# sequential-dexterity/SeqDex

Measured on AMD Instinct MI355X. Metric: env-steps/sec BlockAssemblyGraspSim num_envs=1024/GPU, higher is better.
Workload: dtype f32; 1 GPU; BlockAssemblyGraspSim num_envs=1024 per GPU, fp32, PPO MLP policy [1024,512,256], horizon 8, minibatch_size 4, mini_epochs 5, central value (configs[1]); step=one rl_games epoch = 8 env steps x num_envs + full PPO update, global_envs=1024, piles=synthetic settled piles, 64 per brick-type group, policy=random init, seed 22+rank

## Files before the change

### seqdex_amd/csrc/sdxp_persist.hip

```cpp
#include <cstddef>
#include <cstdlib>

#include "sdx_common.h"
#include "sdxp_device.h"
#include "sdxp_launch.h"
#include "sdxp_persist_lds.h"
#include "sdxp_persist_exchange.h"
#include "sdxp_persist_sums.h"
#include "sdxp_persist_adam.h"
#include "sdxp_persist_tails.h"
#include "sdxp_persist_phase_d.h"

__device__ __forceinline__ const float* obs_rows(const SdxpDev& D, int mb) { return D.mb_obs + (size_t)mb * MB * D.obs_dim; }
__device__ __forceinline__ const float* cvx_rows(const SdxpDev& D, int mb, int mini_epoch) {
  return (mini_epoch == 0 ? D.cvx0 : D.cvx1) + (size_t)mb * MB * ST;
}

template <bool SINGLE>
__global__ __launch_bounds__(NTH, 2) void k_update_persistent(SdxpDev D, int total_steps, const float* gx0_tab, unsigned* failflag, int stamps, int fault) {
  extern __shared__ __attribute__((aligned(16))) char smem_raw[];
  PLds& S = *reinterpret_cast<PLds*>(smem_raw);
  int tid = threadIdx.x, wave = tid >> 6, lane = tid & 63, g = blockIdx.x;
  int r0w, h0, n0, r1w, q1, r1, c2c, c2n, he, hrow, hk;
  auto refresh = [&]() {
    int t = threadIdx.x, b = blockIdx.x;
    asm volatile("" : "+v"(t));
    asm volatile("" : "+s"(b));
    tid = t; lane = t & 63; wave = __builtin_amdgcn_readfirstlane(t >> 6); g = b;
    r0w = wave >> 1; h0 = wave & 1; n0 = 4 * g + r0w;
    r1w = wave >> 2; q1 = wave & 3; r1 = 2 * g + r1w;
    c2c = (t >> 5) & 1; c2n = 32 * (t >> 6) + (t & 31);
    he = HPC * g + t; hrow = he >> 8; hk = he & (U2 - 1);
  };
  refresh();
#define TS(i) if (stamps && g == (stamps >> 8) && tid == 0) { const long long t_ = __builtin_amdgcn_s_memtime(); S.tacc[i] += t_ - S.tlast; S.tlast = t_; }
  if (tid < 32) S.tacc[tid] = 0;
  if (tid == 0) S.fail = 0;
  if (tid == 0) S.tlast = __builtin_amdgcn_s_memtime();
  const int A = ACT;
  u64* const LL = D.ll;
  const __amdgpu_buffer_rsrc_t LQ = lq_rsrc(D.ll);

  float w0a[I0A], m0a[I0A], v0a[I0A], w0c[I0A], m0c[I0A], v0c[I0A], w0v[I0V], m0v[I0V], v0v[I0V];
  float w1[3][4], m1[3][4], v1[3][4];
  float c1[3][4], cm1[3][4], cv1[3][4];
  float w2[3], m2[3], v2[3];
  float c2[3], cm2[3], cv2[3];
  float hw = 0.0f, hm = 0.0f, hv = 0.0f;

  auto ldm = [&](const float* p, size_t o) -> float { return SINGLE ? 0.0f : p[o]; };
  auto P_of = [&](int net) -> float* { return net == 2 ? D.cv : D.ac; };
  auto M_of = [&](int net) -> float* { return net == 2 ? D.cv_m : D.ac_m; };
  auto V_of = [&](int net) -> float* { return net == 2 ? D.cv_v : D.ac_v; };
  auto woff = [&](int net, int l) -> size_t { return net == 0 ? D.off.a_w[l] : net == 1 ? D.off.c_w[l] : D.coff.w[l]; };
  auto boff = [&](int net, int l) -> size_t { return net == 0 ? D.off.a_b[l] : net == 1 ? D.off.c_b[l] : D.coff.b[l]; };
  auto head_woff = [&](int row) -> size_t { return row < A ? D.off.mu_w + (size_t)row * U2 : (row == A ? D.off.v_w : D.coff.v_w); };
  auto head_boff = [&](int row) -> size_t { return row < A ? D.off.mu_b + row : (row == A ? D.off.v_b : D.coff.v_b); };
  auto head_net = [&](int row) -> int { return row < A ? 0 : (row == A ? 1 : 2); };
  auto k_w1 = [&](int i) -> int { return q1 * 256 + lane + 64 * i; };
  auto o_w0 = [&](int net, int k) -> size_t { return woff(net, 0) + (size_t)n0 * D.obs_dim + k; };
  auto o_w1 = [&](int net, int i) -> size_t { return woff(net, 1) + (size_t)r1 * U0 + q1 * 256 + lane + 64 * i; };
  auto o_hw = [&]() -> size_t { return head_woff(hrow) + hk; };

#pragma unroll
  for (int i = 0; i < I0A; ++i) {
    const int kk = lane + 64 * i, k = h0 * H0A + kk;
    const bool ok = kk < H0A && k < D.obs_dim;
    const size_t oa = o_w0(0, k), oc = o_w0(1, k);
    w0a[i] = ok ? D.ac[oa] : 0.0f; m0a[i] = ok ? ldm(D.ac_m, oa) : 0.0f; v0a[i] = ok ? ldm(D.ac_v, oa) : 0.0f;
    w0c[i] = ok ? D.ac[oc] : 0.0f; m0c[i] = ok ? ldm(D.ac_m, oc) : 0.0f; v0c[i] = ok ? ldm(D.ac_v, oc) : 0.0f;
  }
#pragma unroll
  for (int i = 0; i < I0V; ++i) {
    const int kk = lane + 64 * i, k = h0 * H0V + kk;
    const bool ok = kk < H0V;
    const size_t o = woff(2, 0) + (size_t)n0 * ST + k;
    w0v[i] = ok ? D.cv[o] : 0.0f; m0v[i] = ok ? ldm(D.cv_m, o) : 0.0f; v0v[i] = ok ? ldm(D.cv_v, o) : 0.0f;
  }
#pragma unroll
  for (int net = 0; net < 3; ++net) {
#pragma unroll
    for (int i = 0; i < 4; ++i) {
      const size_t o = o_w1(net, i);
      w1[net][i] = P_of(net)[o]; m1[net][i] = ldm(M_of(net), o); v1[net][i] = ldm(V_of(net), o);
    }
#pragma unroll
    for (int c = 0; c < 4; ++c) {
      const size_t o = woff(net, 1) + (size_t)tid * U0 + 4 * g + c;
      c1[net][c] = P_of(net)[o]; cm1[net][c] = ldm(M_of(net), o); cv1[net][c] = ldm(V_of(net), o);
    }
    {
      const size_t o = woff(net, 2) + (size_t)g * U1 + wave * 64 + lane;
      w2[net] = P_of(net)[o]; m2[net] = ldm(M_of(net), o); v2[net] = ldm(V_of(net), o);
    }
    {
      const size_t o = woff(net, 2) + (size_t)c2n * U1 + 2 * g + c2c;
      c2[net] = P_of(net)[o]; cm2[net] = ldm(M_of(net), o); cv2[net] = ldm(V_of(net), o);
    }
  }
  if (tid < HPC) {
    const int net = head_net(hrow);
    const size_t o = o_hw();
    hw = P_of(net)[o]; hm = ldm(M_of(net), o); hv = ldm(V_of(net), o);
  }
  __shared__ float s_b2[3][32];
  auto bias_load = [&](int net, size_t o) { S.bias[tid] = P_of(net)[o]; S.bias_m[tid] = ldm(M_of(net), o); S.bias_v[tid] = ldm(V_of(net), o); };
  if (tid < BIAS_L1) { const int net = (tid - BIAS_L0) / 4, w = (tid - BIAS_L0) % 4; bias_load(net, boff(net, 0) + 4 * g + w); }
  else if (tid < BIAS_L2) { const int net = (tid - BIAS_L1) / 2, r = (tid - BIAS_L1) % 2; bias_load(net, boff(net, 1) + 2 * g + r); }
  else if (tid < BIAS_HEAD) { const int net = tid - BIAS_L2; bias_load(net, boff(net, 2) + g); }
  else if (tid < BIAS_HEAD + A + 2) { const int row = tid - BIAS_HEAD; bias_load(head_net(row), head_boff(row)); }
  else if (tid >= T_LOGSTD && tid < T_LOGSTD + A) {
    const int a = tid - T_LOGSTD;
    const size_t o = D.off.logstd + a;
    s_b2[0][a] = D.ac[o]; s_b2[1][a] = ldm(D.ac_m, o); s_b2[2][a] = ldm(D.ac_v, o);
  }
// ... 9 lines not shown
  float g0a[I0A], g0c[I0A], g0v[I0V];
#pragma unroll
  for (int i = 0; i < I0A; ++i) { g0a[i] = 0.0f; g0c[i] = 0.0f; }
#pragma unroll
  for (int i = 0; i < I0V; ++i) g0v[i] = 0.0f;
  for (int i = tid; i < MB * OBS; i += NTH) (&S.obs[0][0])[i] = 0.0f;
  __syncthreads();

  auto load_rows = [&](int mb_, int me_) {
    auto uni = [](const float* q) -> const float* { unsigned long long a = (unsigned long long)q; asm volatile("" : "+s"(a)); return (const float*)a; };
    const float* o = uni(obs_rows(D, mb_));
    const float* c = uni(cvx_rows(D, mb_, me_));
    const unsigned odim = D.obs_dim;
    if constexpr (!SINGLE) {
      const float* gt = uni(gx0_tab + (size_t)mb_ * GX0_STRIDE);
      if (wave == NWV - 1 && lane < 32)
        __builtin_amdgcn_global_load_lds(SDX_AS_GLOBAL(gt + (lane < 16 ? GX0_OBS + lane : (me_ == 0 ? GX0_CVX0 : GX0_CVX1) + (lane - 16))), SDX_AS_LDS(&S.gx0[0][0]), 4, 0, 0);
    }
    if (odim == OBS) {
      static_assert(offsetof(PLds, cvx) == sizeof(float) * MB * OBS && (MB * OBS) % 4 == 0 && (MB * ST) % 4 == 0, "obs and cvx images are adjacent 16-byte runs");
      constexpr int PO = MB * OBS / 4, PA = PO + MB * ST / 4;
      char* l0 = reinterpret_cast<char*>(&S.obs[0][0]);
#pragma unroll
      for (int j = 0; j < (PA + NTH - 1) / NTH; ++j) {
        const int pc = tid + NTH * j;
        if (pc < PA) {
          const float* src = pc < PO ? o + 4 * pc : c + 4 * (pc - PO);
          __builtin_amdgcn_global_load_lds(SDX_AS_GLOBAL(src), SDX_AS_LDS(l0 + (wave + NWV * j) * 1024), 16, 0, 0);
        }
      }
      return;
    }
#pragma unroll
    for (int s = 0; s < MB; ++s) {
      const float* orow = uni(o + s * odim);
      const float* crow = uni(c + s * ST);
      if ((unsigned)tid < odim) __builtin_amdgcn_global_load_lds(SDX_AS_GLOBAL(orow + (unsigned)tid), SDX_AS_LDS(&S.obs[s][wave * 64]), 4, 0, 0);
      __builtin_amdgcn_global_load_lds(SDX_AS_GLOBAL(crow + (unsigned)tid), SDX_AS_LDS(&S.cvx[s][wave * 64]), 4, 0, 0);
      if (tid + NTH < ST) __builtin_amdgcn_global_load_lds(SDX_AS_GLOBAL(crow + NTH + (unsigned)tid), SDX_AS_LDS(&S.cvx[s][NTH]), 4, 0, 0);
    }
  };
  if (total_steps > 0) load_rows(SINGLE ? gctl->mb_index : 0, SINGLE ? gctl->mini_epoch : 0);
  u32x4 pg0[4];
  bool pg0_issued = false;
  for (int step = 0; step <= total_steps; ++step) {
    SDX_LDS_BARRIER();
    if (S.fail) return;
    if (fault && g == NWG - 1 && step == 3) return;
    refresh();
    const bool last = step == total_steps;
    const int mbi = SINGLE ? gctl->mb_index : step % D.num_minibatches, mini_epoch = SINGLE ? gctl->mini_epoch : step / D.num_minibatches;
    const unsigned tag = tag_base + (unsigned)step + 1u, tag_prev = tag_base + (unsigned)step;
    if (pending) {
      float nr0 = S.n2rest[0], nr1 = S.n2rest[1], nr2 = S.n2rest[2];
      float ac_lr_bc1 = S.scal[SC_AC_LR_BC1], ac_isq = S.scal[SC_AC_ISQ], cv_lr_bc1 = S.scal[SC_CV_LR_BC1], cv_isq = S.scal[SC_CV_ISQ];
      float w0[4], w1[4], w2[4];
      lq_take_or_gather<4>(pg0_issued, pg0, LQ, LQ_G0 + lane, 64, tag_prev, w0, w1, w2, failflag, S.fail);
      float n2[3];
      n2[0] = (w0[0] + w0[1]) + (w0[2] + w0[3]); n2[1] = (w1[0] + w1[1]) + (w1[2] + w1[3]); n2[2] = (w2[0] + w2[1]) + (w2[2] + w2[3]);
#pragma unroll
      for (int net = 0; net < 3; ++net) n2[net] = wave_sum(n2[net]);
      SDX_PIN4X(nr0, nr1, nr2, ac_lr_bc1); SDX_PIN3X(ac_isq, cv_lr_bc1, cv_isq);
      n2[0] += nr0; n2[1] += nr1; n2[2] += nr2;
      const float ac_gn = __builtin_amdgcn_sqrtf(n2[0] + n2[1]), cv_gn = __builtin_amdgcn_sqrtf(n2[2]);
      const float gs_ac = D.truncate_grads ? fminf(1.0f, D.grad_norm * __builtin_amdgcn_rcpf(ac_gn + 1e-6f)) : 1.0f;
      const float gs_cv = D.truncate_grads ? fminf(1.0f, D.grad_norm * __builtin_amdgcn_rcpf(cv_gn + 1e-6f)) : 1.0f;
      if (tid == 0) { S.ctl.ac_gn = ac_gn; S.ctl.cv_gn = cv_gn; S.scal[SC_AC_GSCALE] = gs_ac; S.scal[SC_CV_GSCALE] = gs_cv; }
      TS(0)
#pragma unroll
      for (int i = 0; i < I0A; ++i) {
        adam1p(w0a[i], g0a[i] * gs_ac, m0a[i], v0a[i], ac_lr_bc1, ac_isq);
        adam1p(w0c[i], g0c[i] * gs_ac, m0c[i], v0c[i], ac_lr_bc1, ac_isq);
      }
#pragma unroll
      for (int i = 0; i < I0V; ++i) adam1p(w0v[i], g0v[i] * gs_cv, m0v[i], v0v[i], cv_lr_bc1, cv_isq);
      if (tid < BIAS_L1) {
        const int net = (tid - BIAS_L0) / 4;
        float gg = 0.0f;
        for (int s = 0; s < MB; ++s) gg += S.dyown[net][s][DY_L0 + (tid - BIAS_L0) % 4];
        adam_bias(S, StepScal{gs_ac, gs_cv, ac_lr_bc1, ac_isq, cv_lr_bc1, cv_isq}, tid, net, gg);
      }
      TS(1)
    }
    if (!last) {
      SDX_WAIT_VMCNT0();
      __syncthreads();
      float pa[MB], pc[MB], pv[MB];
#pragma unroll
      for (int s = 0; s < MB; ++s) { pa[s] = 0.0f; pc[s] = 0.0f; pv[s] = 0.0f; }
#pragma unroll
      for (int i = 0; i < I0A; ++i) {
        const int kk = lane + 64 * i, k = h0 * H0A + kk;
        if (kk < H0A) {
#pragma unroll
          for (int s = 0; s < MB; ++s) { const float x = S.obs[s][k]; pa[s] += w0a[i] * x; pc[s] += w0c[i] * x; }
        }
      }
#pragma unroll
      for (int i = 0; i < I0V; ++i) {
        const int kk = lane + 64 * i, k = h0 * H0V + kk;
        if (kk < H0V) {
#pragma unroll
          for (int s = 0; s < MB; ++s) pv[s] += w0v[i] * S.cvx[s][k];
        }
      }
      {
        float v[3 * MB], u[3];
#pragma unroll
        for (int s = 0; s < MB; ++s) { v[0 * MB + s] = pa[s]; v[1 * MB + s] = pc[s]; v[2 * MB + s] = pv[s]; }
        wave_sums<3 * MB>(v, u, lane);
        fpart_store(S, u, wave, lane);
      }
      __syncthreads();
      if (wave == 0) {
        float y[3];
        fwd_tail<0>(S, lane, y);
        if (tid < MB * 4) lq_store(LQ, LQ_X1 + (unsigned)(tid / 4) * U0 + 4 * g + tid % 4, y[0], y[1], y[2], tag);
      }
      TS(2)
    }
    refresh();
    if (pending) {
      const StepScal sc = step_scal(S);
      adam_l1_ahead(S, sc, q1 * 256 + lane, 4 * g, r1w, tid, w1, m1, v1, c1, cm1, cv1, [](int, int, float) {});
      if (tid >= BIAS_L1 && tid < BIAS_L2) {
        const int net = (tid - BIAS_L1) / 2;
        float gg = 0.0f;
        for (int s = 0; s < MB; ++s) gg += S.dyown[net][s][DY_L1 + (tid - BIAS_L1) % 2];
        adam_bias(S, sc, tid, net, gg);
      }
    }
    TS(3)
    if (!last) {
      __syncthreads();
      {
        float v0[8], v1[8], v2[8];
        if (!lq_gather<8>(LQ, LQ_X1 + tid, NTH, tag, v0, v1, v2, failflag)) S.fail = 1;
        image_store(S.x1, v0, v1, v2, tid);
      }
      TS(4)
      __syncthreads();
      {
        float q[3 * MB], u[3];
#pragma unroll
        for (int net = 0; net < 3; ++net) {
#pragma unroll
          for (int s = 0; s < MB; ++s) q[net * MB + s] = 0.0f;
#pragma unroll
          for (int i = 0; i < 4; ++i) {
            const int k = k_w1(i);
#pragma unroll
            for (int s = 0; s < MB; ++s) q[net * MB + s] += w1[net][i] * S.x1[net][s][k];
          }
        }
        wave_sums<3 * MB>(q, u, lane);
        fpart_store(S, u, wave, lane);
      }
      __syncthreads();
      if (wave == 0) {
        float y[3];
        fwd_tail<1>(S, lane, y);
        if (tid < MB * 2) lq_store(LQ, LQ_X2 + (unsigned)(tid / 2) * U1 + 2 * g + tid % 2, y[0], y[1], y[2], tag);
      }
      TS(5)
    }
    refresh();
    u32x4 px2[4];
    bool px2_issued = false;
    if (pending) {
      const StepScal sc = step_scal(S);
      float dep = 0.0f;
#pragma unroll
      for (int net = 0; net < 3; ++net) {
        if (net == 2 && !last) { lq_peek<4>(LQ, LQ_X2 + tid, NTH, px2); px2_issued = true; }
        const float gs = sc.gs(net), lrb = sc.lrb(net), isq = sc.isq(net);
        float d2r[MB], dn2[MB];
        const int o_n = opaque(c2n, dep);
#pragma unroll
        for (int s = 0; s < MB; ++s) { d2r[s] = S.dyown[net][s][DY_L2] * gs; dn2[s] = S.dy2[net][s][o_n] * gs; }
        {
          const int k = opaque(wave * 64 + lane, dep);
          float gg = 0.0f;
#pragma unroll
          for (int s = 0; s < MB; ++s) gg += d2r[s] * S.x2[net][s][k];
          adam1(w2[net], gg, m2[net], v2[net], lrb, isq); dep = w2[net];
        }
        {
          const int k = opaque(2 * g + c2c, dep);
          float gg = 0.0f;
#pragma unroll
          for (int s = 0; s < MB; ++s) gg += dn2[s] * S.x2[net][s][k];
          adam1(c2[net], gg, cm2[net], cv2[net], lrb, isq); dep = c2[net];
        }
      }
      if (tid < HPC) {
        const int net = head_net(hrow);
        const float gs = sc.gs(net), lrb = sc.lrb(net), isq = sc.isq(net);
        float gg = 0.0f;
#pragma unroll
        for (int s = 0; s < MB; ++s) gg += (hrow < A ? S.dmu[s][hrow] : S.dv[hrow - A][s]) * gs * S.x3[net][s][hk];
        adam1(hw, gg, hm, hv, lrb, isq);
        ll_store(LL + LL_HW + he, hw, tag_prev);
      }
      if (tid >= BIAS_L2 && tid < BIAS_HEAD + A + 2) {
        int net; float gg = 0.0f;
        if (tid < BIAS_HEAD) { net = tid - BIAS_L2; for (int s = 0; s < MB; ++s) gg += S.dyown[net][s][DY_L2]; }
        else { const int row = tid - BIAS_HEAD; net = head_net(row); for (int s = 0; s < MB; ++s) gg += row < A ? S.dmu[s][row] : S.dv[row - A][s]; }
        adam_bias(S, sc, tid, net, gg);
      } else if (tid >= T_LOGSTD && tid < T_LOGSTD + A) {
        const int a = tid - T_LOGSTD;
        float b = s_b2[0][a], bm = s_b2[1][a], bv = s_b2[2][a];
        adam1(b, S.dls[a] * sc.gs(0), bm, bv, sc.lrb(0), sc.isq(0));
        s_b2[0][a] = b; s_b2[1][a] = bm; s_b2[2][a] = bv;
      }
    }
    TS(6)
    if (last) break;
    __syncthreads();
    const size_t r0 = (size_t)mbi * MB;
    float pf_act = 0.0f, pf_omu = 0.0f, pf_osg = 1.0f;
    float pf_adv = 0.0f, pf_nlp = 0.0f, pf_ret = 0.0f, pf_val = 0.0f;
    if (tid < MB * 32 && (tid % 32) == 31) {
      const size_t i = r0 + tid / 32;
      pf_adv = D.adv[i]; pf_nlp = D.mb_neglogp[i];
    }
    if (tid >= T_VLOSS && tid < T_VLOSS + 2 * MB) {
      const size_t i = r0 + (tid - T_VLOSS) % MB;
      pf_ret = D.returns[i]; pf_val = D.mb_values[i];
    }
    if (tid < MB * 32 && (tid % 32) < A) {
      const size_t i = (r0 + tid / 32) * A + tid % 32;
      pf_act = D.mb_actions[i];
      pf_omu = __hip_atomic_load(&D.mb_mus[i], __ATOMIC_RELAXED, __HIP_MEMORY_SCOPE_AGENT);
      pf_osg = __hip_atomic_load(&D.mb_sigmas[i], __ATOMIC_RELAXED, __HIP_MEMORY_SCOPE_AGENT);
    }
    {
      static_assert(NTH == U1 && MB == 4, "word tid + NTH j of the x2 edge is (sample j, unit tid)");
      float x[3][MB], u[3];
      {
        float v0[4], v1[4], v2[4];
        lq_take_or_gather<4>(px2_issued, px2, LQ, LQ_X2 + tid, NTH, tag, v0, v1, v2, failflag, S.fail);
        TS(7)
#pragma unroll
        for (int s = 0; s < MB; ++s) { x[0][s] = v0[s]; x[1][s] = v1[s]; x[2][s] = v2[s]; }
        image_store(S.x2, v0, v1, v2, tid);
      }
      fwd2_sums(w2, x, u, lane);
      fwd2_store(S, u, wave, lane);
    }
    __syncthreads();
    if (wave == 0) {
      float y[3];
      fwd_tail<2>(S, lane, y);
      if (tid < MB) lq_store(LQ, LQ_X3 + (unsigned)tid * U2 + g, y[0], y[1], y[2], tag);
    }
    TS(8)
    if (tid < MB * 32) { S.act[tid / 32][tid % 32] = pf_act; S.omu[tid / 32][tid % 32] = pf_omu; S.osg[tid / 32][tid % 32] = pf_osg; }
    if (tid >= T_LS && tid < T_LS + 32) { const float l_ = (tid - T_LS < A) ? s_b2[0][tid - T_LS] : 0.0f; S.ls[tid - T_LS] = l_; S.sgm[tid - T_LS] = expf(l_); }
    if constexpr (!SINGLE)
    {
      float ua[8], ub[8];
      {
        float p[30];
#pragma unroll
        for (int i = 0; i < 30; ++i) p[i] = 0.0f;
#pragma unroll
        for (int net = 0; net < 3; ++net) gram_acc10(&p[net * 10], S.x2[net][0][tid], S.x2[net][1][tid], S.x2[net][2][tid], S.x2[net][3][tid]);
        row_butterfly<30>(p, ua, lane);
      }
      rows_store<8>(S, ua, 0, wave, lane);
      {
        float p[30];
#pragma unroll
        for (int i = 0; i < 30; ++i) p[i] = 0.0f;
#pragma unroll
        for (int h = 0; h < U0 / NTH; ++h) {
#pragma unroll
          for (int net = 0; net < 3; ++net) { const int k = tid + NTH * h; gram_acc10(&p[net * 10], S.x1[net][0][k], S.x1[net][1][k], S.x1[net][2][k], S.x1[net][3][k]); }
          if (h == 0) {
#pragma unroll
            for (int i = 0; i < 30; ++i) asm("" : "+v"(p[i]));
          }
        }
        row_butterfly<30>(p, ub, lane);
      }
      rows_store<8>(S, ub, 32, wave, lane);
      rows_reduce(S, 64, S.part, tid);
      if (tid < 48) S.gx[tid >> 4][2][tid & 15] = S.part[(tid >> 4) * 10 + tri16(tid & 15)];
      else if (tid >= 64 && tid < 64 + 48) { const int t = tid - 64; S.gx[t >> 4][1][t & 15] = S.part[32 + (t >> 4) * 10 + tri16(t & 15)]; }
    }
    TS(9)
    refresh();
    float wh[HR][4];
    bool row_done = false;
    {
      u32x4 w3[2];
#pragma unroll
      for (int i = 0; i < 2; ++i) w3[i] = load16(LQ, LQ_X3 + tid + i * NTH);
      if (step != 0) {
        u64 ww[HR][4];
        const u64 absent = (u64)tag_prev << 32;
#pragma unroll
        for (int j = 0; j < HR; ++j) {
          const int row = wave + 8 * j;
#pragma unroll
          for (int e = 0; e < 4; ++e)
            ww[j][e] = row < A + 2 ? __hip_atomic_load(LL + LL_HW + (size_t)row * U2 + lane + 64 * e, __ATOMIC_RELAXED, __HIP_MEMORY_SCOPE_AGENT) : absent;
        }
        bool ok = true;
#pragma unroll
        for (int j = 0; j < HR; ++j)
#pragma unroll
          for (int e = 0; e < 4; ++e) ok = ok && (unsigned)(ww[j][e] >> 32) == tag_prev;
        if (__builtin_amdgcn_ballot_w64(!ok) == 0) {
#pragma unroll
          for (int j = 0; j < HR; ++j)
#pragma unroll
            for (int e = 0; e < 4; ++e) wh[j][e] = __uint_as_float((unsigned)ww[j][e]);
          row_done = true;
        }
      }
      float v0[2], v1[2], v2[2];
#pragma unroll
      for (int i = 0; i < 2; ++i) { v0[i] = __uint_as_float(w3[i].x); v1[i] = __uint_as_float(w3[i].y); v2[i] = __uint_as_float(w3[i].z); }
      if (__builtin_amdgcn_ballot_w64(!(lq_ok(w3[0], tag) && lq_ok(w3[1], tag))) != 0) {
        if (!lq_gather<2>(LQ, LQ_X3 + tid, NTH, tag, v0, v1, v2, failflag)) S.fail = 1;
      }
      image_store(S.x3, v0, v1, v2, tid);
    }
    if (!row_done) {
#pragma unroll
    for (int j = 0; j < HR; ++j) {
      const int row = wave + 8 * j;
#pragma unroll
      for (int e = 0; e < 4; ++e) wh[j][e] = 0.0f;
      if (row < A + 2) {
        if (step == 0) {
          const float* hp = P_of(head_net(row)) + head_woff(row) + lane;
#pragma unroll
          for (int e = 0; e < 4; ++e) wh[j][e] = hp[64 * e];
        } else if (!ll_gather<4>(LL + LL_HW + (size_t)row * U2 + lane, 64, tag_prev, wh[j], failflag)) S.fail = 1;
      }
    }
    }
    TS(10)
    __syncthreads();
    head_forward(S, wh, wave, lane);
    __syncthreads();
    TS(11)
    SDX_OPAQUE(pf_adv); SDX_OPAQUE(pf_nlp); SDX_OPAQUE(pf_ret); SDX_OPAQUE(pf_val);
    ZOps zo;
    loss_request(S, tid, zo);
    __builtin_amdgcn_sched_barrier(0);
    float wc[13];
    if (step == 0) {
#pragma unroll
      for (int j = 0; j < 13; ++j) { const int row = min(13 * c2c + j, A + 1); wc[j] = P_of(head_net(row))[head_woff(row) + c2n]; }
    } else {
      const unsigned* hwv = reinterpret_cast<const unsigned*>(LL + LL_HW) + 2 * c2n;
#pragma unroll
      for (int j = 0; j < 13; ++j) {
        const int row = min(13 * c2c + j, A + 1);
        wc[j] = __uint_as_float(__hip_atomic_load(hwv + (size_t)row * (2 * U2), __ATOMIC_RELAXED, __HIP_MEMORY_SCOPE_AGENT));
      }
    }
    const float invM = 1.0f / (float)MB;
    {
      const LossCfg lc = {D.e_clip, D.critic_coef, D.bounds_coef, (bool)D.clip_value};
      float q, bt;
      loss_front(S, lc, tid, zo, pf_adv, pf_nlp, pf_ret, pf_val, invM, q, bt);
      SDX_LDS_BARRIER();
      loss_back(S, tid, q, bt, invM);
      if (g == 0 && tid < MB * 32 && tid % 32 < A) {
        const int s = tid / 32, a = tid % 32;
        __hip_atomic_store(&D.mb_mus[(r0 + s) * A + a], S.mu[s][a], __ATOMIC_RELAXED, __HIP_MEMORY_SCOPE_AGENT);
        __hip_atomic_store(&D.mb_sigmas[(r0 + s) * A + a], S.sgm[a], __ATOMIC_RELAXED, __HIP_MEMORY_SCOPE_AGENT);
      }
      SDX_LDS_BARRIER();
    }
    TS(12)
    refresh();
    float d2[3][MB];
    head_backward(S, wc, c2c, c2n, d2);
    TS(13)
    {
      float p[12];
#pragma unroll
      for (int net = 0; net < 3; ++net)
#pragma unroll
        for (int s = 0; s < MB; ++s) p[net * MB + s] = d2[net][s] * c2[net];
#pragma unroll
      for (int net = 0; net < 3; ++net)
#pragma unroll
        for (int i = 0; i < 2; ++i) {
          float lo = d2[net][i], hi = d2[net][2 + i];
          asm volatile("" : "+v"(lo), "+v"(hi));
          S.dy2[net][2 * c2c + i][c2n] = c2c ? hi : lo;
        }
      {
        float u2[3];
        row_butterfly<12>(p, u2, lane);
        rows_store<3>(S, u2, 0, wave, lane);
      }
      const int bi = tid >> 1, bc = tid & 1, bnet = min(tid >> 3, 2), bs = bi & 3;
      const float eg = tid < 24 ? elu_g(S.x2[bnet][bs][2 * g + bc]) : 0.0f;
      SDX_LDS_BARRIER();
      if (wave == 0) {
        float v = 0.0f;
        if (tid < 24) {
          float r[2 * NWV];
#pragma unroll
          for (int w = 0; w < NWV; ++w) { r[2 * w] = S.red[4 * w + 2 * bc][bi]; r[2 * w + 1] = S.red[4 * w + 2 * bc + 1][bi]; }
          asm volatile("" ::: "memory");
          float t = 0.0f;
#pragma unroll
          for (int j = 0; j < 2 * NWV; ++j) t += r[j];
          v = t * eg;
          S.dyown[bnet][bs][DY_L1 + bc] = v;
        }
        const float v1 = dpp_mov<0x108, 0xF>(0.0f, v);
        const unsigned y = __builtin_bit_cast(unsigned, v);
        const auto r = __builtin_amdgcn_permlane16_swap(y, y, false, false);
        const float v2 = __builtin_bit_cast(float, (unsigned)r[1]);
        if (tid < MB * 2) lq_store(LQ, LQ_DY1 + (unsigned)(tid >> 1) * U1 + 2 * g + (tid & 1), v, v1, v2, tag);
      }
    }
    TS(14)
    u32x4 pdy1[4];
    bool pdy1_issued = false;
    if (wave == 5 || wave == 7) {
      const int s = (wave - 5) + (lane >> 5), a = lane & 31;
      float r_kl = 0.0f, r_bl = 0.0f, r_ent = 0.0f;
      if (a < A) {
        const float ls = S.ls[a], sg = S.sgm[a], mu = S.mu[s][a];
        const float omu = S.omu[s][a], osg = S.osg[s][a];
        r_kl = logf(osg / sg + 1e-5f) + (sg * sg + (omu - mu) * (omu - mu)) / (2.0f * (osg * osg + 1e-5f)) - 0.5f;
        const float hi = fmaxf(mu - 1.1f, 0.0f), lo = fminf(mu + 1.1f, 0.0f);
        r_bl = hi * hi + lo * lo;
        r_ent = 0.5f + 0.5f * 1.8378770664093453f + ls;
      }
      r_kl = half_sum(r_kl); r_bl = half_sum(r_bl); r_ent = half_sum(r_ent);
      if (a == 31) { S.stat[s][STAT_BOUNDS] = r_bl; S.stat[s][STAT_KL] = r_kl; S.stat[s][STAT_ENTROPY] = r_ent; }
    }
    if (tid == T_STATS) {
      PLds::Ctl& C = S.ctl;
      C.ac_lr_applied = C.ac_lr;
      if constexpr (!SINGLE) {
        C.ac_t += 1; C.cv_t += 1;
        C.ac_b1 *= 0.9; C.ac_b2 *= 0.999; C.cv_b1 *= 0.9; C.cv_b2 *= 0.999;
        S.scal[SC_AC_LR_BC1] = C.ac_lr_applied / (float)(1.0 - C.ac_b1); S.scal[SC_AC_ISQ] = 1.0f / sqrtf((float)(1.0 - C.ac_b2));
        S.scal[SC_CV_LR_BC1] = C.cv_lr / (float)(1.0 - C.cv_b1); S.scal[SC_CV_ISQ] = 1.0f / sqrtf((float)(1.0 - C.cv_b2));
      }
    }
    auto stats_and_lr = [&]() { if (tid == T_STATS) stats_lr_once(S, invM, D.adaptive_lr, D.kl_threshold); };
    if constexpr (SINGLE) { SDX_LDS_BARRIER(); stats_and_lr(); }
    if constexpr (!SINGLE) {
      float p[30];
#pragma unroll
      for (int i = 0; i < 30; ++i) p[i] = 0.0f;
      if (tid >= T_HEAD_G && tid < T_HEAD_G + 48) {
        const int t = tid - T_HEAD_G, net = t / 16, a = (t / 4) % 4, b = t % 4;
        float dd = 0.0f;
        if (net == 0) { for (int j = 0; j < A; ++j) dd += S.dmu[a][j] * S.dmu[b][j]; }
        else dd = S.dv[net - 1][a] * S.dv[net - 1][b];
        S.part[PART_HEAD_G + t] = dd;
// ... 330 lines not shown
```

### seqdex_amd/csrc/sdxp_persist_checks.hip

```cpp
#include "sdx_common.h"
#include "sdxp_launch.h"
#include "sdxp_persist_sums.h"
#include "sdxp_persist_adam.h"
#include "sdxp_persist_tails.h"
#include "sdxp_persist_phase_d.h"

template <int N>
__global__ __launch_bounds__(NTH) void k_wave_sums_check(const float* in, float* ref, float* got) {
  const int tid = threadIdx.x, lane = tid & 63;
  float v[N], u[(N + 3) / 4];
#pragma unroll
  for (int i = 0; i < N; ++i) v[i] = in[i * NTH + tid];
#pragma unroll
  for (int i = 0; i < N; ++i) ref[i * NTH + tid] = wave_sum(v[i]);
  wave_sums<N>(v, u, lane);
#pragma unroll
  for (int j = 0; j < (N + 3) / 4; ++j) got[(4 * j + (lane & 3)) * NTH + tid] = u[j];
}
extern "C" int sdxpk_wave_sums_check(const float* in, float* ref, float* got, int n, hipStream_t st) {
  if (n == 12) hipLaunchKernelGGL(k_wave_sums_check<12>, dim3(1), dim3(NTH), 0, st, in, ref, got);
  else if (n == 16) hipLaunchKernelGGL(k_wave_sums_check<16>, dim3(1), dim3(NTH), 0, st, in, ref, got);
  else return -1;
  return hipGetLastError() == hipSuccess ? 0 : -1;
}
__global__ __launch_bounds__(NTH) void k_fwd2_sums_check(const float* w, const float* x, float* ref, float* got) {
  const int tid = threadIdx.x, lane = tid & 63;
  float wv[3], xv[3][MB], u[3];
#pragma unroll
  for (int net = 0; net < 3; ++net) {
    wv[net] = w[net * NTH + tid];
#pragma unroll
    for (int s = 0; s < MB; ++s) xv[net][s] = x[(net * MB + s) * NTH + tid];
  }
#pragma unroll
  for (int net = 0; net < 3; ++net)
#pragma unroll
    for (int s = 0; s < MB; ++s) {
      float t = wv[net] * xv[net][s];
      asm volatile("" : "+v"(t));
      float v = __builtin_fmaf(wv[net], xv[net][s], dpp_mov<0xB1, 0xF>(0.0f, t));
      v = dpp_add<0x4E, 0xF>(v); v = dpp_add<0x141, 0xF>(v); v = dpp_add<0x140, 0xF>(v); v = dpp_add<0x142, 0xA>(v); v = dpp_add<0x143, 0xC>(v);
      ref[(net * MB + s) * NTH + tid] = __builtin_bit_cast(float, __builtin_amdgcn_readlane(__builtin_bit_cast(int, v), 63));
    }
  fwd2_sums(wv, xv, u, lane);
  if ((0xA5A5 >> (lane & 15)) & 1) {
    const int s = fwd2_sample(lane);
#pragma unroll
    for (int net = 0; net < 3; ++net) got[(net * MB + s) * NTH + tid] = u[net];
  }
}
extern "C" int sdxpk_fwd2_sums_check(const float* w, const float* x, float* ref, float* got, hipStream_t st) {
  hipLaunchKernelGGL(k_fwd2_sums_check, dim3(1), dim3(NTH), 0, st, w, x, ref, got);
  return hipGetLastError() == hipSuccess ? 0 : -1;
}
__global__ __launch_bounds__(NTH) void k_input_grams_reference(const float* obs, int obs_dim, const float* cvx, float* out) {
  extern __shared__ __attribute__((aligned(16))) char smem_raw[];
  PLds& S = *reinterpret_cast<PLds*>(smem_raw);
  const int tid = threadIdx.x, wave = tid >> 6, lane = tid & 63;
  const size_t mb = blockIdx.x;
  for (int i = tid; i < MB * OBS; i += NTH) { const int s = i / OBS, k = i % OBS; S.obs[s][k] = k < obs_dim ? obs[(mb * MB + s) * obs_dim + k] : 0.0f; }
  for (int i = tid; i < MB * ST; i += NTH) (&S.cvx[0][0])[i] = cvx[mb * MB * ST + i];
  __syncthreads();
  float p[22];
#pragma unroll
  for (int i = 0; i < 22; ++i) p[i] = 0.0f;
  if (tid < OBS) gram_acc10(&p[0], S.obs[0][tid], S.obs[1][tid], S.obs[2][tid], S.obs[3][tid]);
  gram_acc10(&p[11], S.cvx[0][tid], S.cvx[1][tid], S.cvx[2][tid], S.cvx[3][tid]);
  if (tid + NTH < ST) gram_acc10(&p[11], S.cvx[0][tid + NTH], S.cvx[1][tid + NTH], S.cvx[2][tid + NTH], S.cvx[3][tid + NTH]);
  block_sum<22>(S, p, S.part, tid, wave, lane);
  if (tid < 16) out[mb * 32 + tid] = S.part[tri16(tid)];
  else if (tid >= 64 && tid < 80) out[mb * 32 + 16 + tid - 64] = S.part[11 + tri16(tid - 64)];
}
extern "C" int sdxpk_input_grams_reference(const float* obs, int obs_dim, const float* cvx, int n_mb, float* out, hipStream_t st) {
  if (obs_dim < 1 || obs_dim > OBS || n_mb < 1) return -1;
  if (hipFuncSetAttribute(reinterpret_cast<const void*>(k_input_grams_reference), hipFuncAttributeMaxDynamicSharedMemorySize, (int)sizeof(PLds)) != hipSuccess) return -1;
  hipLaunchKernelGGL(k_input_grams_reference, dim3(n_mb), dim3(NTH), sizeof(PLds), st, obs, obs_dim, cvx, out);
  return hipGetLastError() == hipSuccess ? 0 : -1;
}
__global__ __launch_bounds__(NTH) void k_adam_ahead_check(const float* x1, const float* dy1, const float* dyr, const float* scal, int g, const float* state, float* out) {
  extern __shared__ __attribute__((aligned(16))) char smem_raw[];
  PLds& S = *reinterpret_cast<PLds*>(smem_raw);
  const int tid = threadIdx.x, wave = tid >> 6, lane = tid & 63, r1w = wave >> 2, q1 = wave & 3;
  for (int i = tid; i < 3 * MB * U0; i += NTH) (&S.x1[0][0][0])[i] = x1[i];
  for (int i = tid; i < 3 * MB * U1; i += NTH) (&S.dy1[0][0][0])[i] = dy1[i];
// ... 453 lines not shown
  };
  fill();
  {
    float pf_adv = 0.0f, pf_nlp = 0.0f, pf_ret = 0.0f, pf_val = 0.0f;
    if (tid < MB * 32 && (tid % 32) == 31) { const int i = tid / 32; pf_adv = ps[i]; pf_nlp = ps[MB + i]; pf_ret = ps[2 * MB + i]; pf_val = ps[3 * MB + i]; }
    SDX_OPAQUE(pf_adv); SDX_OPAQUE(pf_nlp); SDX_OPAQUE(pf_ret); SDX_OPAQUE(pf_val);
    {
      float r_nlp = 0.0f;
      if (tid < MB * 32) {
        const int s = tid / 32, a = tid % 32;
        const float zz = (a < A) ? (S.act[s][a] - S.mu[s][a]) / S.sgm[a] : 0.0f;
        S.z[s][a] = zz;
        if (a < A) r_nlp = 0.5f * zz * zz + S.ls[a];
      }
      r_nlp = half_sum(r_nlp);
      if (tid < MB * 32 && (tid % 32) == 31) {
        const int s = tid / 32;
        const float nlp = r_nlp + 0.5f * 1.8378770664093453f * (float)A;
        const float adv = pf_adv;
        const float ratio = expf(pf_nlp - nlp);
        const float L1 = -adv * ratio, L2 = -adv * clampf(ratio, 1.0f - D.e_clip, 1.0f + D.e_clip);
        const bool inr = ratio >= 1.0f - D.e_clip && ratio <= 1.0f + D.e_clip;
        S.gnlp[s] = (L1 > L2 || inr) ? adv * ratio : 0.0f;
        const float R = pf_ret, vo = pf_val;
        float closs[2];
        for (int j = 0; j < 2; ++j) {
          const float v = S.val[j][s];
          const float vc = vo + clampf(v - vo, -D.e_clip, D.e_clip);
          const float c1v = (v - R) * (v - R), c2v = (vc - R) * (vc - R);
          float d;
          if (D.clip_value) {
            closs[j] = fmaxf(c1v, c2v);
            const bool inv = fabsf(v - vo) <= D.e_clip;
            d = (c1v > c2v || inv) ? 2.0f * (v - R) : 0.0f;
          } else { closs[j] = c1v; d = 2.0f * (v - R); }
          S.dv[j][s] = (j == 0 ? 0.5f * D.critic_coef : 1.0f) * d * invM;
        }
        S.stat[s][STAT_ACTOR] = fmaxf(L1, L2); S.stat[s][STAT_CRITIC] = closs[0]; S.stat[s][STAT_CV] = closs[1];
      }
    }
    SDX_LDS_BARRIER();
    if (tid < MB * 32) {
      const int s = tid / 32, a = tid % 32;
      float dmu = 0.0f;
      if (a < A) {
        const float sg = S.sgm[a], mu = S.mu[s][a];
        const float hi = fmaxf(mu - 1.1f, 0.0f), lo = fminf(mu + 1.1f, 0.0f);
        dmu = S.gnlp[s] * (-(S.z[s][a] / sg)) * invM + D.bounds_coef * (2.0f * hi + 2.0f * lo) * invM;
      }
      S.dmu[s][a] = dmu;
    }
    if (tid >= T_LS && tid < T_LS + 32) {
      const int a = tid - T_LS;
      float dls = 0.0f;
      if (a < A) for (int s = 0; s < MB; ++s) dls += S.gnlp[s] * (1.0f - S.z[s][a] * S.z[s][a]) * invM;
      S.dls[a] = dls;
    }
    SDX_LDS_BARRIER();
  }
  copy_out(out + c * 2 * LOSS_OUT);
  fill();
  {
    float pf_adv = 0.0f, pf_nlp = 0.0f, pf_ret = 0.0f, pf_val = 0.0f;
    if (tid < MB * 32 && (tid % 32) == 31) { const int i = tid / 32; pf_adv = ps[i]; pf_nlp = ps[MB + i]; }
    if (tid >= T_VLOSS && tid < T_VLOSS + 2 * MB) { const int i = (tid - T_VLOSS) % MB; pf_ret = ps[2 * MB + i]; pf_val = ps[3 * MB + i]; }
    SDX_OPAQUE(pf_adv); SDX_OPAQUE(pf_nlp); SDX_OPAQUE(pf_ret); SDX_OPAQUE(pf_val);
    ZOps zo;
    loss_request(S, tid, zo);
    const LossCfg lc = {D.e_clip, D.critic_coef, D.bounds_coef, (bool)D.clip_value};
    float q, bt;
    loss_front(S, lc, tid, zo, pf_adv, pf_nlp, pf_ret, pf_val, invM, q, bt);
    SDX_LDS_BARRIER();
    loss_back(S, tid, q, bt, invM);
    SDX_LDS_BARRIER();
  }
  copy_out(out + c * 2 * LOSS_OUT + LOSS_OUT);
}
extern "C" int sdxpk_loss_phase_check(const float* in, int n, float* out, hipStream_t st) {
  if (n < 1) return -1;
  if (hipFuncSetAttribute(reinterpret_cast<const void*>(k_loss_phase_check), hipFuncAttributeMaxDynamicSharedMemorySize, (int)sizeof(PLds)) != hipSuccess) return -1;
  hipLaunchKernelGGL(k_loss_phase_check, dim3(n), dim3(NTH), sizeof(PLds), st, in, out);
  return hipGetLastError() == hipSuccess ? 0 : -1;
}
```

### seqdex_amd/csrc/sdxp_persist_exchange.h

```cpp
#pragma once
#include "sdx_common.h"
#include "sdxp_types.h"
#include "sdxp_persist_lds.h"
#include "sdxp_tagged_words.h"

namespace {
typedef unsigned long long u64;
constexpr unsigned LQ_X1 = 0, LQ_X2 = LQ_X1 + MB * U0, LQ_X3 = LQ_X2 + MB * U1, LQ_DY1 = LQ_X3 + MB * U2, LQ_DY0 = LQ_DY1 + MB * U1,
                   LQ_G0 = LQ_DY0 + MB * U0, LQ_END = LQ_G0 + 16 * NWG;
constexpr size_t LL_HW = 2 * (size_t)LQ_END, LL_END = LL_HW + (ACT + 2) * U2;
static_assert(LL_END <= SDXP_LL_WORDS, "exchange buffer too small");
__device__ __forceinline__ __amdgpu_buffer_rsrc_t lq_rsrc(void* ll) { return __builtin_amdgcn_make_buffer_rsrc(ll, 0, SDXP_LL_WORDS * 8, 0x00020000); }
template <int N>
__device__ __forceinline__ void lq_peek(__amdgpu_buffer_rsrc_t q, unsigned idx0, unsigned stride, u32x4 (&w)[N]) {
#pragma unroll
  for (int i = 0; i < N; ++i) w[i] = load16(q, idx0 + i * stride);
}
template <int N>
__device__ __forceinline__ bool lq_take(const u32x4 (&w)[N], unsigned tag, float (&o0)[N], float (&o1)[N], float (&o2)[N]) {
  bool ok = true;
#pragma unroll
  for (int i = 0; i < N; ++i) ok = ok && lq_ok(w[i], tag);
#pragma unroll
  for (int i = 0; i < N; ++i) { o0[i] = __uint_as_float(w[i].x); o1[i] = __uint_as_float(w[i].y); o2[i] = __uint_as_float(w[i].z); }
  return __builtin_amdgcn_ballot_w64(!ok) == 0;
}
template <int N>
__device__ __forceinline__ bool lq_gather(__amdgpu_buffer_rsrc_t q, unsigned idx0, unsigned stride, unsigned tag, float (&o0)[N], float (&o1)[N], float (&o2)[N],
                                          unsigned* failflag) {
  unsigned spins = 0;
  for (;;) {
    u32x4 w[N];
#pragma unroll
    for (int i = 0; i < N; ++i) w[i] = __builtin_amdgcn_raw_buffer_load_b128(q, (idx0 + i * stride) * 16u, 0, 16);
    bool ok = true;
#pragma unroll
    for (int i = 0; i < N; ++i) ok = ok && lq_ok(w[i], tag);
#pragma unroll
    for (int i = 0; i < N; ++i) { o0[i] = __uint_as_float(w[i].x); o1[i] = __uint_as_float(w[i].y); o2[i] = __uint_as_float(w[i].z); }
    if (__builtin_amdgcn_ballot_w64(!ok) == 0) return true;
    SDX_POLL_SLEEP_OR_GIVE_UP(spins, failflag)
  }
}
template <int N>
__device__ __forceinline__ void lq_take_or_gather(bool issued, const u32x4 (&pw)[N], __amdgpu_buffer_rsrc_t q, unsigned idx0, unsigned stride, unsigned tag, float (&o0)[N],
                                          float (&o1)[N], float (&o2)[N], unsigned* failflag, int& fail) {
  if (!(issued && lq_take<N>(pw, tag, o0, o1, o2)) && !lq_gather<N>(q, idx0, stride, tag, o0, o1, o2, failflag)) fail = 1;
}
template <int N, int U>
__device__ __forceinline__ void image_store(float (&img)[3][MB][U], const float (&v0)[N], const float (&v1)[N], const float (&v2)[N], int tid) {
  static_assert(N * NTH == MB * U, "N words per thread cover the image");
#pragma unroll
  for (int j = 0; j < N; ++j) { (&img[0][0][0])[tid + NTH * j] = v0[j]; (&img[1][0][0])[tid + NTH * j] = v1[j]; (&img[2][0][0])[tid + NTH * j] = v2[j]; }
}
__device__ __forceinline__ void ll_store(u64* p, float v, unsigned tag) {
  __hip_atomic_store(p, ((u64)tag << 32) | (u64)__float_as_uint(v), __ATOMIC_RELAXED, __HIP_MEMORY_SCOPE_AGENT);
}
template <int N>
__device__ __forceinline__ bool ll_gather(const u64* p, size_t stride, unsigned tag, float (&out)[N], unsigned* failflag) {
  unsigned spins = 0;
  for (;;) {
    u64 w[N];
#pragma unroll
    for (int i = 0; i < N; ++i) w[i] = __hip_atomic_load(p + i * stride, __ATOMIC_RELAXED, __HIP_MEMORY_SCOPE_AGENT);
    bool ok = true;
#pragma unroll
    for (int i = 0; i < N; ++i) ok = ok && (unsigned)(w[i] >> 32) == tag;
#pragma unroll
    for (int i = 0; i < N; ++i) out[i] = __uint_as_float((unsigned)w[i]);
    if (__builtin_amdgcn_ballot_w64(!ok) == 0) return true;
    SDX_POLL_SLEEP_OR_GIVE_UP(spins, failflag)
  }
}
}
```

Measured before the change: 40140 env-steps/s.

## Pack head weights into tagged 16-byte exchange words and prefetch them earlier

Head-layer weights were published as one tagged 64-bit word per element. They are now packed three rows per 16-byte tagged line via DPP and permlane swaps, with row 24 kept as separate tagged words. Readers peek these packed lines early, overlapped with the Gram reductions, and load the column view with wide buffer loads. The goal is fewer atomic loads and stores and less polling latency on the cross-CU head exchange. In exchange it adds a new ownership mapping, an extra waitcnt, and test kernels, and relies on layout assumptions enforced by static_asserts.

```diff
diff --git a/seqdex_amd/csrc/sdxp_persist.hip b/seqdex_amd/csrc/sdxp_persist.hip
--- a/seqdex_amd/csrc/sdxp_persist.hip
+++ b/seqdex_amd/csrc/sdxp_persist.hip
@@ -30,7 +30,7 @@
     r0w = wave >> 1; h0 = wave & 1; n0 = 4 * g + r0w;
     r1w = wave >> 2; q1 = wave & 3; r1 = 2 * g + r1w;
     c2c = (t >> 5) & 1; c2n = 32 * (t >> 6) + (t & 31);
-    he = HPC * g + t; hrow = he >> 8; hk = he & (U2 - 1);
+    head_owned(b, t, he, hrow, hk);
   };
   refresh();
 #define TS(i) if (stamps && g == (stamps >> 8) && tid == 0) { const long long t_ = __builtin_amdgcn_s_memtime(); S.tacc[i] += t_ - S.tlast; S.tlast = t_; }
@@ -206,6 +206,7 @@
       }
       TS(1)
     }
+    __builtin_amdgcn_s_waitcnt(0x0F70);
     if (!last) {
       SDX_WAIT_VMCNT0();
       __syncthreads();
@@ -324,8 +325,8 @@
 #pragma unroll
         for (int s = 0; s < MB; ++s) gg += (hrow < A ? S.dmu[s][hrow] : S.dv[hrow - A][s]) * gs * S.x3[net][s][hk];
         adam1(hw, gg, hm, hv, lrb, isq);
-        ll_store(LL + LL_HW + he, hw, tag_prev);
-      }
+      }
+      if (wave == 0) head_publish(LQ, LL, tid, he, hw, tag_prev);
       if (tid >= BIAS_L2 && tid < BIAS_HEAD + A + 2) {
         int net; float gg = 0.0f;
         if (tid < BIAS_HEAD) { net = tid - BIAS_L2; for (int s = 0; s < MB; ++s) gg += S.dyown[net][s][DY_L2]; }
@@ -381,6 +382,8 @@
     TS(8)
     if (tid < MB * 32) { S.act[tid / 32][tid % 32] = pf_act; S.omu[tid / 32][tid % 32] = pf_omu; S.osg[tid / 32][tid % 32] = pf_osg; }
     if (tid >= T_LS && tid < T_LS + 32) { const float l_ = (tid - T_LS < A) ? s_b2[0][tid - T_LS] : 0.0f; S.ls[tid - T_LS] = l_; S.sgm[tid - T_LS] = expf(l_); }
+    u32x4 ph[4];
+    u64 p24[4];
     if constexpr (!SINGLE)
     {
       float ua[8], ub[8];
@@ -409,6 +412,7 @@
         row_butterfly<30>(p, ub, lane);
       }
       rows_store<8>(S, ub, 32, wave, lane);
+      head_rows_peek(LQ, wave, lane, ph); head_row24_peek(LL, wave, lane, tag_prev, p24);
       rows_reduce(S, 64, S.part, tid);
       if (tid < 48) S.gx[tid >> 4][2][tid & 15] = S.part[(tid >> 4) * 10 + tri16(tid & 15)];
       else if (tid >= 64 && tid < 64 + 48) { const int t = tid - 64; S.gx[t >> 4][1][t & 15] = S.part[32 + (t >> 4) * 10 + tri16(t & 15)]; }
@@ -422,27 +426,8 @@
 #pragma unroll
       for (int i = 0; i < 2; ++i) w3[i] = load16(LQ, LQ_X3 + tid + i * NTH);
       if (step != 0) {
-        u64 ww[HR][4];
-        const u64 absent = (u64)tag_prev << 32;
-#pragma unroll
-        for (int j = 0; j < HR; ++j) {
-          const int row = wave + 8 * j;
-#pragma unroll
-          for (int e = 0; e < 4; ++e)
-            ww[j][e] = row < A + 2 ? __hip_atomic_load(LL + LL_HW + (size_t)row * U2 + lane + 64 * e, __ATOMIC_RELAXED, __HIP_MEMORY_SCOPE_AGENT) : absent;
-        }
-        bool ok = true;
-#pragma unroll
-        for (int j = 0; j < HR; ++j)
-#pragma unroll
-          for (int e = 0; e < 4; ++e) ok = ok && (unsigned)(ww[j][e] >> 32) == tag_prev;
-        if (__builtin_amdgcn_ballot_w64(!ok) == 0) {
-#pragma unroll
-          for (int j = 0; j < HR; ++j)
-#pragma unroll
-            for (int e = 0; e < 4; ++e) wh[j][e] = __uint_as_float((unsigned)ww[j][e]);
-          row_done = true;
-        }
+        if constexpr (SINGLE) { head_rows_peek(LQ, wave, lane, ph); head_row24_peek(LL, wave, lane, tag_prev, p24); }
+        row_done = head_rows_take(ph, p24, tag_prev, wh);
       }
       float v0[2], v1[2], v2[2];
 #pragma unroll
@@ -453,19 +438,19 @@
       image_store(S.x3, v0, v1, v2, tid);
     }
     if (!row_done) {
-#pragma unroll
-    for (int j = 0; j < HR; ++j) {
-      const int row = wave + 8 * j;
-#pragma unroll
-      for (int e = 0; e < 4; ++e) wh[j][e] = 0.0f;
-      if (row < A + 2) {
-        if (step == 0) {
-          const float* hp = P_of(head_net(row)) + head_woff(row) + lane;
-#pragma unroll
-          for (int e = 0; e < 4; ++e) wh[j][e] = hp[64 * e];
-        } else if (!ll_gather<4>(LL + LL_HW + (size_t)row * U2 + lane, 64, tag_prev, wh[j], failflag)) S.fail = 1;
-      }
-    }
+      if (step == 0) {
+#pragma unroll
+        for (int j = 0; j < HR; ++j) {
+          const int row = wave + 8 * j;
+#pragma unroll
+          for (int e = 0; e < 4; ++e) wh[j][e] = 0.0f;
+          if (row < A + 2) {
+            const float* hp = P_of(head_net(row)) + head_woff(row) + lane;
+#pragma unroll
+            for (int e = 0; e < 4; ++e) wh[j][e] = hp[64 * e];
+          }
+        }
+      } else if (!head_rows_gather(LQ, LL, wave, lane, tag_prev, wh, failflag)) S.fail = 1;
     }
     TS(10)
     __syncthreads();
@@ -476,18 +461,15 @@
     ZOps zo;
     loss_request(S, tid, zo);
     __builtin_amdgcn_sched_barrier(0);
-    float wc[13];
+    HeadCols hc;
     if (step == 0) {
 #pragma unroll
-      for (int j = 0; j < 13; ++j) { const int row = min(13 * c2c + j, A + 1); wc[j] = P_of(head_net(row))[head_woff(row) + c2n]; }
-    } else {
-      const unsigned* hwv = reinterpret_cast<const unsigned*>(LL + LL_HW) + 2 * c2n;
-#pragma unroll
-      for (int j = 0; j < 13; ++j) {
-        const int row = min(13 * c2c + j, A + 1);
-        wc[j] = __uint_as_float(__hip_atomic_load(hwv + (size_t)row * (2 * U2), __ATOMIC_RELAXED, __HIP_MEMORY_SCOPE_AGENT));
-      }
-    }
+      for (int w = 0; w < 8; ++w) {
+        const int ra = w + 8 * c2c, rb = ra + 8;
+        hc.pair[w].x = __float_as_uint(P_of(head_net(ra))[head_woff(ra) + c2n]); hc.pair[w].y = __float_as_uint(P_of(head_net(rb))[head_woff(rb) + c2n]);
+      }
+      hc.r24 = __float_as_uint(P_of(2)[head_woff(A + 1) + c2n]);
+    } else head_cols_load(LQ, c2c, c2n, hc);
     const float invM = 1.0f / (float)MB;
     {
       const LossCfg lc = {D.e_clip, D.critic_coef, D.bounds_coef, (bool)D.clip_value};
@@ -505,6 +487,8 @@
     TS(12)
     refresh();
     float d2[3][MB];
+    float wc[13];
+    head_cols_take(hc, c2c, wc);
     head_backward(S, wc, c2c, c2n, d2);
     TS(13)
     {
diff --git a/seqdex_amd/csrc/sdxp_persist_checks.hip b/seqdex_amd/csrc/sdxp_persist_checks.hip
--- a/seqdex_amd/csrc/sdxp_persist_checks.hip
+++ b/seqdex_amd/csrc/sdxp_persist_checks.hip
@@ -1,5 +1,6 @@
 #include "sdx_common.h"
 #include "sdxp_launch.h"
+#include "sdxp_persist_exchange.h"
 #include "sdxp_persist_sums.h"
 #include "sdxp_persist_adam.h"
 #include "sdxp_persist_tails.h"
@@ -619,3 +620,43 @@
   hipLaunchKernelGGL(k_loss_phase_check, dim3(n), dim3(NTH), sizeof(PLds), st, in, out);
   return hipGetLastError() == hipSuccess ? 0 : -1;
 }
+__global__ __launch_bounds__(64) void k_head_publish_check(const float* W, unsigned tag, int stale_cu, u64* ll, int* own) {
+  const int t = threadIdx.x, g = blockIdx.x;
+  int he, hrow, hk;
+  head_owned(g, t, he, hrow, hk);
+  float hw = 0.0f;
+  if (t < HPC) { hw = W[hrow * U2 + hk]; own[(g * HPC + t) * 2] = hrow; own[(g * HPC + t) * 2 + 1] = hk; }
+  head_publish(lq_rsrc(ll), ll, t, he, hw, g == stale_cu ? tag - 1u : tag);
+}
+__global__ __launch_bounds__(NTH) void k_head_views_check(u64* ll, unsigned tag, float* wh_out, float* wc_out, int* verdict) {
+  const int tid = threadIdx.x, lane = tid & 63, wave = __builtin_amdgcn_readfirstlane(tid >> 6);
+  const __amdgpu_buffer_rsrc_t q = lq_rsrc(ll);
+  u32x4 ph[4];
+  u64 p24[4];
+  float wh[HR][4];
+  head_rows_peek(q, wave, lane, ph);
+  head_row24_peek(ll, wave, lane, tag, p24);
+  const bool hit = head_rows_take(ph, p24, tag, wh);
+  if (lane == 0) verdict[wave] = hit ? 1 : 0;
+#pragma unroll
+  for (int j = 0; j < HR; ++j)
+#pragma unroll
+    for (int e = 0; e < 4; ++e) wh_out[(tid * HR + j) * 4 + e] = wh[j][e];
+  const int c2c = (tid >> 5) & 1, c2n = 32 * (tid >> 6) + (tid & 31);
+  HeadCols hc;
+  float wc[13];
+  head_cols_load(q, c2c, c2n, hc);
+  head_cols_take(hc, c2c, wc);
+#pragma unroll
+  for (int j = 0; j < 13; ++j) wc_out[tid * 13 + j] = wc[j];
+}
+extern "C" size_t sdxpk_head_words_ll_words() { return SDXP_LL_WORDS; }
+extern "C" int sdxpk_head_publish_check(const float* W, unsigned tag, int stale_cu, unsigned long long* ll, int* own, hipStream_t st) {
+  if (stale_cu >= NWG) return -1;
+  hipLaunchKernelGGL(k_head_publish_check, dim3(NWG), dim3(64), 0, st, W, tag, stale_cu, ll, own);
+  return hipGetLastError() == hipSuccess ? 0 : -1;
+}
+extern "C" int sdxpk_head_views_check(unsigned long long* ll, unsigned tag, float* wh, float* wc, int* verdict, hipStream_t st) {
+  hipLaunchKernelGGL(k_head_views_check, dim3(1), dim3(NTH), 0, st, ll, tag, wh, wc, verdict);
+  return hipGetLastError() == hipSuccess ? 0 : -1;
+}
diff --git a/seqdex_amd/csrc/sdxp_persist_exchange.h b/seqdex_amd/csrc/sdxp_persist_exchange.h
--- a/seqdex_amd/csrc/sdxp_persist_exchange.h
+++ b/seqdex_amd/csrc/sdxp_persist_exchange.h
@@ -2,13 +2,17 @@
 #include "sdx_common.h"
 #include "sdxp_types.h"
 #include "sdxp_persist_lds.h"
+#include "sdxp_persist_sums.h"
 #include "sdxp_tagged_words.h"
 
 namespace {
 typedef unsigned long long u64;
 constexpr unsigned LQ_X1 = 0, LQ_X2 = LQ_X1 + MB * U0, LQ_X3 = LQ_X2 + MB * U1, LQ_DY1 = LQ_X3 + MB * U2, LQ_DY0 = LQ_DY1 + MB * U1,
                    LQ_G0 = LQ_DY0 + MB * U0, LQ_END = LQ_G0 + 16 * NWG;
-constexpr size_t LL_HW = 2 * (size_t)LQ_END, LL_END = LL_HW + (ACT + 2) * U2;
+constexpr unsigned LQ_HW = LQ_END, LQ_HW_END = LQ_HW + 8 * U2;
+constexpr size_t LL_H24 = 2 * (size_t)LQ_HW_END, LL_END = LL_H24 + U2;
+static_assert(ACT + 2 == 3 * 8 + 1 && NWV == 8 && NWG == U2, "three rows per word and wave, row 24 one column per CU");
+static_assert(LQ_HW % 8 == 0, "a CU's eight head words are one 128-byte line");
 static_assert(LL_END <= SDXP_LL_WORDS, "exchange buffer too small");
 __device__ __forceinline__ __amdgpu_buffer_rsrc_t lq_rsrc(void* ll) { return __builtin_amdgcn_make_buffer_rsrc(ll, 0, SDXP_LL_WORDS * 8, 0x00020000); }
 template <int N>
@@ -72,4 +76,58 @@
     SDX_POLL_SLEEP_OR_GIVE_UP(spins, failflag)
   }
 }
+__device__ __forceinline__ void head_owned(int g, int t, int& he, int& hrow, int& hk) {
+  const bool r24 = t >= HPC - 1;
+  hrow = r24 ? ACT + 1 : (g >> 5) + 8 * (t >> 3);
+  hk = r24 ? g : 8 * (g & 31) + (t & 7);
+  he = r24 ? g : 8 * g + (t & 7);
 }
+__device__ __forceinline__ void head_publish(__amdgpu_buffer_rsrc_t q, u64* ll, int t, int he, float hw, unsigned tag) {
+  const float v1 = dpp_mov<0x108, 0xF>(0.0f, hw);
+  const unsigned y = __builtin_bit_cast(unsigned, hw);
+  const auto r = __builtin_amdgcn_permlane16_swap(y, y, false, false);
+  const float v2 = __builtin_bit_cast(float, (unsigned)r[1]);
+  if (t < 8) lq_store(q, LQ_HW + (unsigned)he, hw, v1, v2, tag);
+  else if (t == HPC - 1) ll_store(ll + LL_H24 + he, hw, tag);
+}
+__device__ __forceinline__ unsigned head_row_word(int wave, int lane) { return LQ_HW + 256u * (unsigned)wave + (unsigned)lane; }
+__device__ __forceinline__ void head_rows_peek(__amdgpu_buffer_rsrc_t q, int wave, int lane, u32x4 (&ph)[4]) { lq_peek<4>(q, head_row_word(wave, lane), 64, ph); }
+__device__ __forceinline__ void head_row24_peek(const u64* ll, int wave, int lane, unsigned tag, u64 (&p24)[4]) {
+#pragma unroll
+  for (int e = 0; e < 4; ++e)
+    p24[e] = wave == 0 ? __hip_atomic_load(ll + LL_H24 + lane + 64 * e, __ATOMIC_RELAXED, __HIP_MEMORY_SCOPE_AGENT) : (u64)tag << 32;
+}
+__device__ __forceinline__ bool head_rows_take(const u32x4 (&ph)[4], const u64 (&p24)[4], unsigned tag, float (&wh)[HR][4]) {
+  bool ok = true;
+#pragma unroll
+  for (int e = 0; e < 4; ++e) ok = ok && (unsigned)(p24[e] >> 32) == tag;
+#pragma unroll
+  for (int e = 0; e < 4; ++e) wh[3][e] = __uint_as_float((unsigned)p24[e]);
+  const bool ok3 = lq_take<4>(ph, tag, wh[0], wh[1], wh[2]);
+  return __builtin_amdgcn_ballot_w64(!ok) == 0 && ok3;
+}
+__device__ __forceinline__ bool head_rows_gather(__amdgpu_buffer_rsrc_t q, const u64* ll, int wave, int lane, unsigned tag, float (&wh)[HR][4], unsigned* failflag) {
+  bool ok = lq_gather<4>(q, head_row_word(wave, lane), 64, tag, wh[0], wh[1], wh[2], failflag);
+#pragma unroll
+  for (int e = 0; e < 4; ++e) wh[3][e] = 0.0f;
+  if (wave == 0) ok = ll_gather<4>(ll + LL_H24 + lane, 64, tag, wh[3], failflag) && ok;
+  return ok;
+}
+typedef unsigned int u32x2 __attribute__((ext_vector_type(2)));
+struct HeadCols { u32x2 pair[8]; unsigned r24; };
+__device__ __forceinline__ void head_cols_load(__amdgpu_buffer_rsrc_t q, int c2c, int c2n, HeadCols& hc) {
+  const unsigned v = (LQ_HW + (unsigned)c2n) * 16u + 4u * (unsigned)c2c;
+#pragma unroll
+  for (int w = 0; w < 8; ++w) hc.pair[w] = __builtin_amdgcn_raw_buffer_load_b64(q, v, 4096 * w, 16);
+  hc.r24 = __builtin_amdgcn_raw_buffer_load_b32(q, ((unsigned)LL_H24 + (unsigned)c2n) * 8u, 0, 16);
+}
+__device__ __forceinline__ void head_cols_take(const HeadCols& hc, int c2c, float (&wc)[13]) {
+  static_assert(ACT + 2 == 25, "rows 0..12 and 13..24");
+#pragma unroll
+  for (int j = 0; j < 13; ++j) {
+    const unsigned lo = j < 8 ? hc.pair[j].x : hc.pair[j - 8].y;
+    const unsigned hi = j < 3 ? hc.pair[5 + j].x : (j < 11 ? hc.pair[j - 3].y : hc.r24);
+    wc[j] = __uint_as_float(c2c ? hi : lo);
+  }
+}
+}
```

Result: faster. 42340 env-steps/s, median of 6 (+5.5%).
